# moskewcz/boda

Measured on AMD Instinct MI355X. Metric: effective TFLOP/s (2*M*N*K / time), whole job, higher is better.
Workload: dtype f32

## Files before the change

boda_amd/csrc/kernels/sgemm_big_f32.hip:

```cpp

#ifndef __HIPCC_RTC__
#include <hip/hip_runtime.h>
#endif

typedef float f32x16 __attribute__((ext_vector_type(16)));
typedef float f32x4 __attribute__((ext_vector_type(4)));
typedef unsigned u32x2 __attribute__((ext_vector_type(2)));
#ifndef GROUP_I
#define GROUP_I 8
#endif
#ifndef BKS
#define BKS 8
#endif
#ifndef PF
#define PF 2
#endif
#ifndef TBI
#define TBI 256
#endif
#ifndef TBJ
#define TBJ 256
#endif
#ifndef WI
#define WI 2
#endif
#ifndef WJ
#define WJ 4
#endif
#ifndef MINW
#define MINW 1
#endif
#ifndef MULPRIO
#define MULPRIO 1
#endif
#ifndef STGPRIO
#define STGPRIO 0
#endif
#ifndef NSTG
#define NSTG 4
#endif

struct gemm_args_t {
  float const *I; float const *J; float *D; float const *bias;
  int Mi, Nj, K;
  int ldI, ldJ, ldD;
  int C, H, W, OH, OW;
  int tiles_i, tiles_j;
  int splitk, kt_per;
  float *ws; long ws_slab;
  unsigned I_bytes, J_bytes;
  unsigned D_bytes;
  int out_ctot, out_coff;
  int const *ktab; int ktab_n;
  long bsI, bsJ, bsD;
};

namespace {
constexpr int kNMW = WI * WJ;
static_assert(kNMW == 8 || kNMW == 4, "eight (or four) multiplying waves");
constexpr int kTI = TBI / (WI * 32), kTJ = TBJ / (WJ * 32);
static_assert(TBI % (WI * 32) == 0 && TBJ % (WJ * 32) == 0 && (kTI == 4 || kTI == 2 || kTI == 1) && (kTJ == 2 || kTJ == 1), "wave tile: 4 | 2 | 1 row blocks x 2 | 1 column blocks");
constexpr int kLDI = TBI + 4, kLDJ = TBJ + 4;
constexpr int kImgI = BKS * kLDI, kImgJ = BKS * kLDJ, kImg2 = kImgI + kImgJ;
constexpr int kNLI = BKS * (TBI / 4) / 256, kNLJ = BKS * (TBJ / 4) / 256;
static_assert((BKS * (TBI / 4)) % 256 == 0 && (BKS * (TBJ / 4)) % 256 == 0, "whole float4 units per staging thread");
constexpr int kKK = BKS / 2;
constexpr int kU = (NSTG == 3) ? 3 * PF : ((PF > NSTG) ? PF : NSTG);
constexpr int kD = NSTG - 1;
static_assert(NSTG == 3 || NSTG == 4, "NSTG: 3 | 4");
constexpr int kOOB = (int)0x80000000;
static_assert(BKS % 4 == 0 && (PF == 2 || PF == 4), "BKS % 4 == 0, PF: 2 | 4");
typedef __amdgpu_buffer_rsrc_t rsrc_t;
__device__ __forceinline__ rsrc_t make_rsrc(float const *p, unsigned bytes) { return __builtin_amdgcn_make_buffer_rsrc((void *)p, 0, (int)bytes, 0x00020000); }
__device__ __forceinline__ f32x4 bload4(rsrc_t r, int voff, int soff) { return __builtin_bit_cast(f32x4, __builtin_amdgcn_raw_buffer_load_b128(r, voff, soff, 0)); }
}

#if (TBI / (WI * 32)) == 4
typedef f32x4 avec_t;
#elif (TBI / (WI * 32)) == 2
typedef float2 avec_t;
#else
typedef float avec_t;
#endif
#if (TBJ / (WJ * 32)) == 2
typedef float2 bvec_t;
#else
typedef float bvec_t;
#endif
namespace {
__device__ __forceinline__ float vget(f32x4 const &v, int i) { return v[i]; }
__device__ __forceinline__ float vget(float2 const &v, int i) { return i ? v.y : v.x; }
__device__ __forceinline__ float vget(float const &v, int) { return v; }
}

extern "C" __global__ __launch_bounds__((kNMW + 4) * 64, MINW) void KNAME(gemm_args_t const p) {
  __shared__ __attribute__((aligned(16))) float sm[NSTG * kImg2];
  int const lane = threadIdx.x & 63;
  int const wave = __builtin_amdgcn_readfirstlane(threadIdx.x >> 6);
  bool const stager = wave >= kNMW;

  int tile_i, tile_j;
  {
    int const bid = blockIdx.x, nb = p.tiles_i * p.tiles_j;
    int const q = nb >> 3, rr = nb & 7, xcd = bid & 7, idx = bid >> 3;
    int const nid = ((xcd < rr) ? xcd * (q + 1) : rr * (q + 1) + (xcd - rr) * q) + idx;
    int const group_sz = GROUP_I * p.tiles_j, gid = nid / group_sz, first_i = gid * GROUP_I;
    int const gsz = min(p.tiles_i - first_i, GROUP_I), in_g = nid - gid * group_sz;
    tile_i = first_i + in_g % gsz; tile_j = in_g / gsz;
  }
  int const i0 = tile_i * TBI, j0 = tile_j * TBJ;
  int const nkt = (p.K + BKS - 1) / BKS;
  int const nkt_pad = (nkt + kU - 1) / kU * kU;

  if (stager) {
#if STGPRIO
    __builtin_amdgcn_s_setprio(STGPRIO);
#endif
    int const tid = threadIdx.x - kNMW * 64;
    rsrc_t const rI = make_rsrc(p.I, p.I_bytes), rJ = make_rsrc(p.J, p.J_bytes);
    int goffI[kNLI], goffJ[kNLJ], loffI[kNLI], loffJ[kNLJ], krowI[kNLI], krowJ[kNLJ];
#pragma unroll
    for (int n = 0; n < kNLI; ++n) {
      int const c = tid + n * 256, kr = c / (TBI / 4), x = 4 * (c % (TBI / 4));
      krowI[n] = kr; loffI[n] = kr * kLDI + x;
      goffI[n] = (i0 + x < p.Mi) ? ((kr * p.ldI + i0 + x) * 4) : kOOB;
    }
#pragma unroll
    for (int n = 0; n < kNLJ; ++n) {
      int const c = tid + n * 256, kr = c / (TBJ / 4), x = 4 * (c % (TBJ / 4));
      krowJ[n] = kr; loffJ[n] = kImgI + kr * kLDJ + x;
      goffJ[n] = (j0 + x < p.Nj) ? ((kr * p.ldJ + j0 + x) * 4) : kOOB;
// ... 26 lines not shown
#pragma unroll
        for (int n = 0; n < kNLJ; ++n) { lstoreJ(n, (u + kD) % NSTG, ringJ[(u + kD) % PF][n]); ringJ[(u + kD) % PF][n] = gloadJ(n, kb + u + kD + PF); }
        asm volatile("s_waitcnt lgkmcnt(%0)\n s_barrier" :: "n"(kNLI + kNLJ) : "memory");
      }
    }
    return;
  }

#if MULPRIO
  __builtin_amdgcn_s_setprio(MULPRIO);
#endif
  int const wi = wave / WJ, wj = wave % WJ;
  float const *const a_base = sm + (lane >> 5) * kLDI + wi * (kTI * 32) + kTI * (lane & 31);
  float const *const b_base = sm + kImgI + (lane >> 5) * kLDJ + wj * (kTJ * 32) + kTJ * (lane & 31);
  f32x16 acc[kTI][kTJ];
#pragma unroll
  for (int t = 0; t < kTI; ++t)
#pragma unroll
    for (int u = 0; u < kTJ; ++u)
#pragma unroll
      for (int r = 0; r < 16; ++r) acc[t][u][r] = 0.f;

  asm volatile("s_barrier" ::: "memory");
  avec_t a[2]; bvec_t b[2];
  a[0] = *reinterpret_cast<avec_t const *>(a_base); b[0] = *reinterpret_cast<bvec_t const *>(b_base);
  static_assert(kKK % 2 == 0, "an even number of k pairs per step (the operand double buffer carries over from step to step)");
  for (int kb = 0; kb < nkt_pad; kb += kU) {
#pragma unroll
    for (int s = 0; s < kU; ++s) {
      float const *const A = a_base + (s % NSTG) * kImg2, *const B = b_base + (s % NSTG) * kImg2;
      float const *const An = a_base + ((s + 1) % NSTG) * kImg2, *const Bn = b_base + ((s + 1) % NSTG) * kImg2;
#pragma unroll
      for (int kk = 0; kk < kKK; ++kk) {
        if (kk + 1 < kKK) { a[(kk + 1) & 1] = *reinterpret_cast<avec_t const *>(A + (kk + 1) * 2 * kLDI); b[(kk + 1) & 1] = *reinterpret_cast<bvec_t const *>(B + (kk + 1) * 2 * kLDJ); }
#if NSTG == 4
        else { a[0] = *reinterpret_cast<avec_t const *>(An); b[0] = *reinterpret_cast<bvec_t const *>(Bn); }
#endif
        __builtin_amdgcn_sched_barrier(0);
        avec_t const ca = a[kk & 1]; bvec_t const cb = b[kk & 1];
#pragma unroll
        for (int t = 0; t < kTI; ++t)
#pragma unroll
          for (int u = 0; u < kTJ; ++u) acc[t][u] = __builtin_amdgcn_mfma_f32_32x32x2f32(vget(ca, t), vget(cb, u), acc[t][u], 0, 0, 0);
        __builtin_amdgcn_sched_barrier(0);
      }
#if NSTG == 4
      asm volatile("s_barrier" ::: "memory");
#else
      asm volatile("s_waitcnt lgkmcnt(0)\n s_barrier" ::: "memory");
      a[0] = *reinterpret_cast<avec_t const *>(An); b[0] = *reinterpret_cast<bvec_t const *>(Bn);
#endif
    }
  }

  {
    rsrc_t const rD = make_rsrc(p.D, p.D_bytes);
    int const j = j0 + wj * (kTJ * 32) + kTJ * (lane & 31);
    int const il = i0 + wi * (kTI * 32) + kTI * 4 * (lane >> 5);
#pragma unroll
    for (int t = 0; t < kTI; ++t)
#pragma unroll
      for (int r = 0; r < 16; ++r) {
        int const i = il + kTI * ((r & 3) + 8 * (r >> 2)) + t;
        int const off = ((i < p.Mi) && (j < p.Nj)) ? ((i * p.ldD + j) * 4) : kOOB;
#if (TBJ / (WJ * 32)) == 2
        float2 const v = float2{acc[t][0][r], acc[t][1][r]};
        __builtin_amdgcn_raw_buffer_store_b64(__builtin_bit_cast(u32x2, v), rD, off, 0, 0);
#else
        float const v = acc[t][0][r];
        __builtin_amdgcn_raw_buffer_store_b32(__builtin_bit_cast(unsigned, v), rD, off, 0, 0);
#endif
      }
  }
}
```

boda_amd/csrc/native_internal.h:

```cpp
#pragma once
#include "native_kernels.h"
#include <algorithm>
#include <cstdlib>
#include <sstream>

namespace bodahip {

struct gemm_args_t {
  float const *I; float const *J; float *D; float const *bias;
  int Mi, Nj, K;
  int ldI, ldJ, ldD;
  int C, H, W, OH, OW;
  int tiles_i, tiles_j;
  int splitk, kt_per;
  float *ws; long ws_slab;
  unsigned I_bytes, J_bytes;
  unsigned D_bytes;
  int out_ctot, out_coff;
  void const *ktab; int ktab_n;
  long bsI, bsJ, bsD;
};
struct chain_args_t : gemm_args_t {
  float const *I2; float const *bias2; float *Dmid;
  int M2; unsigned I2_bytes, Dmid_bytes;
};
static_assert(sizeof(gemm_args_t) == 176, "gemm_args_t is declared with this size by every kernel source (and by set_kernel_source's text)");

struct kernel_t { hipModule_t mod = nullptr; hipFunction_t func = nullptr; int occ = 0; };

struct native_kernels_t::impl_t {
  std::map<string, kernel_t> kernels;
  std::map<string, string> tune;
  void *ws = nullptr; size_t ws_bytes = 0;
  bool ws_used = false;
  std::vector<void *> ws_retired;
// ... 62 lines not shown
  float *w0; float *w1; float *w2; float *w3;
  float *ws;
  float *outs[8];
  long n;
  int B, C, HW, N;
  int slab, nslabs;
  int quads;
  int step_img, step_pel;
  float fN, eps, maf, omm, unb;
};
static_assert(sizeof(bn_args_t) == 13 * 8 + 8 * 8 + 8 + 9 * 4 + 5 * 4, "bn_args_t is declared with this layout by kernels/bn_f32.hip");
struct bn_launch_t { plan_t p; int op = 0; };
struct bn_plan_t { std::vector<bn_launch_t> ls; double algo_bytes = 0; size_t ws_bytes = 0; };
bn_plan_t plan_bn(bn_op_t const &b);
string bn_plan_desc(bn_op_t const &b, bn_plan_t const &bp);

struct rows_args_t {
  void const *filts; void const *in; void *out; float const *bias;
  int n_img, oc; unsigned filts_bytes, in_bytes, out_bytes; int out_ctot, out_coff; int n_chunks, rows_per_chunk; float lrn_alpha, lrn_beta, lrn_k;
};

struct sgemm_split_t { uint32_t m_main = 0; string tail_tile; double t_single = 0, t_split = 0; };
static char const *const kBigTile = "256x256x16x2x4x1x1x32x2";
struct sgemm_part_t { uint32_t m0 = 0, rows = 0, n0 = 0, cols = 0; string tile; };
struct set_member_in_t { conv_geom_t g; bool patch_filts, pool; int grp_pad; };
struct set_layout_t { std::vector<int> in_set, alone, variant_of; std::vector<plan_t const *> variants; std::vector<string> vkeys; int minw = 8; string skey; };

extern char const *const k_src_conv_nhwc_bf16_ptr, *const k_src_conv_nhwc_patch_bf16_ptr, *const k_src_winograd_f32_ptr;
bool parse_tile(string const &s, tile_cfg_t &c);
void launch(native_host_t *host, kernel_t &k, gemm_args_t &a, tile_cfg_t const &c);
plan_t plan_sgemm(uint32_t M, uint32_t N, uint32_t K, int num_cus, string const &tile, bool bf16 = false, int batch = 1, bool allow_big = true);
bool plan_patch_bf16(conv_geom_t const &g, int num_cus, plan_t &p);
plan_t plan_conv_nhwc(conv_geom_t const &g, int num_cus, string const &tile, bool out_f32, int grp_pad = 0, bool allow_split = true, bool res = false);
plan_t plan_conv_nhwc_patch(conv_geom_t const &g, int num_cus, string const &tile_arg, bool out_f32, bool pool = false);
bool plan_conv_nhwc_rows(conv_geom_t const &g, post_ops_t const &post, int num_cus, plan_t &p, string *why = nullptr);
bool rows_auto(conv_geom_t const &g, int num_cus, string const &tile);
bool apply_post_ops(op_base_t const &op, conv_geom_t &g, post_ops_t &post, char const *what);
bool plan_ipconv_dma(conv_geom_t const &g, int num_cus, plan_t &p);
plan_t plan_conv(conv_geom_t const &g, int num_cus, string const &tile, bool bf16 = false, string const &k1s = string(), bool allow_splitk = true, bool exact = true);
plan_t plan_bconv_in(conv_geom_t const &g, int num_cus, string const &tile, bool zinp = false);
plan_t plan_bconv_filts(conv_geom_t const &g, int num_cus, string const &tile);
plan_t plan_bconv_filts_biases(conv_geom_t const &g, int num_cus, string const &tile);
plan_t plan_bconv_in_bf16(conv_geom_t const &g, int num_cus, string const &tile, bool zinp = false);
plan_t plan_bconv_fb_bf16(conv_geom_t const &g, int num_cus, string const &tile);
plan_t plan_bconv_slab_sum();
plan_t plan_bconv_biases();
long bconv_in_tiles(conv_geom_t const &g, int BJ);
// ... 22 lines not shown
```

boda_amd/csrc/native_kernels.cc:

```cpp
#include "native_internal.h"

namespace bodahip {

#include "kernels_embed.inc"

native_kernels_t::native_kernels_t(native_host_t *host_) : impl(new impl_t), host(host_) {
  if (char const *e = getenv("BODAHIP_SGEMM_TILE")) impl->tune["sgemm_tile"] = e;
  if (char const *e = getenv("BODAHIP_CONV_TILE")) impl->tune["conv_tile"] = e;
  if (char const *e = getenv("BODAHIP_K1_STREAM")) impl->tune["k1_stream"] = e;
  if (char const *e = getenv("BODAHIP_CONV_ALGO")) impl->tune["conv_algo"] = e;
  if (char const *e = getenv("BODAHIP_EXACT")) impl->tune["exact"] = e;
}
native_kernels_t::~native_kernels_t() {
  if (impl->ts_bytes && impl->ws) {
    char const *e = getenv("BODAHIP_CBIG_TSTAMP"); string fn = e ? string(e) : string(); if (fn.size() > 5 && fn.substr(fn.size() - 5) == ":late") fn.resize(fn.size() - 5);
    std::vector<unsigned long long> h(impl->ts_bytes / 8);
    if (!fn.empty() && hipDeviceSynchronize() == hipSuccess && hipMemcpy(h.data(), (char *)impl->ws + impl->ts_off, impl->ts_bytes, hipMemcpyDeviceToHost) == hipSuccess) {
      if (FILE *f = fopen(fn.c_str(), "a")) { fprintf(f, "%s\n", impl->ts_hdr.c_str());
        for (size_t w = 0; w < h.size() / 16; ++w) { for (int e2 = 0; e2 < 16; ++e2) fprintf(f, "%llu ", h[w * 16 + e2]); fprintf(f, "\n"); } fclose(f); }
    }
  }
  for (auto &kv : impl->kernels) { if (kv.second.mod) (void)hipModuleUnload(kv.second.mod); }
  if (impl->wino_mod) (void)hipModuleUnload(impl->wino_mod);
  if (impl->ws) (void)hipFree(impl->ws);
// ... 185 lines not shown
}

static ktab_t get_rtab(native_kernels_t::impl_t *impl, native_host_t *host, conv_geom_t const &g) {
  string const key = "rows:" + std::to_string(g.C) + "," + std::to_string(g.H) + "," + std::to_string(g.W) + "," + std::to_string(g.KH);
  long const R = (long)g.C * g.KH, n = ((R + 63) / 64 + 1) * 64;
  auto it = impl->ktabs.find(key);
  if (it != impl->ktabs.end()) return ktab_t{it->second, (int)n};
  if (host->nh_capturing()) rt_err("graph capture: gather table not built yet -- run the call list once before capturing it");
  std::vector<int> h((size_t)n * 2);
  for (long r = 0; r < n; ++r) {
    if (r < R) { long const ic = r / g.KH, ky = r % g.KH; h[r] = (int)((ic * g.H + ky) * g.W); h[n + r] = (int)ky; }
    else { h[r] = 0; h[n + r] = 1 << 30; }
  }
  void *d = nullptr;
  hip_err_chk(hipMalloc(&d, h.size() * sizeof(int)), "hipMalloc(rtab)");
  hip_err_chk(hipMemcpyAsync(d, h.data(), h.size() * sizeof(int), hipMemcpyHostToDevice, host->nh_stream()), "hipMemcpyAsync(rtab)");
  hip_err_chk(hipStreamSynchronize(host->nh_stream()), "hipStreamSynchronize");
  impl->ktabs.emplace(key, d);
  return ktab_t{d, (int)n};
}

string tune_of(native_kernels_t::impl_t *impl, char const *key) { auto t = impl->tune.find(key); return (t == impl->tune.end()) ? string() : t->second; }

static void sgemm_parts(native_kernels_t *nk, native_kernels_t::impl_t *impl, native_host_t *host, float const *a, float const *b, float *c, uint32_t M, uint32_t N, uint32_t K, std::vector<sgemm_part_t> const &parts) {
  if ((uint64_t)K * M * 4 > 0x80000000ull || (uint64_t)K * N * 4 > 0x80000000ull || (uint64_t)M * N * 4 >= 0x7ffffff0ull) unsup_err("hip_sgemm: operands / c of 2 GiB or more are not supported (32-bit buffer offsets)");
  uint32_t grid = 0; bool first = true;
  for (sgemm_part_t const &q : parts) {
    plan_t const p = plan_sgemm(q.rows, q.cols, K, host->nh_num_cus(), q.tile, false);
    kernel_t &k = get_kernel(impl, host, p);
    gemm_args_t ga; memset(&ga, 0, sizeof(ga));
    ga.I = a + q.m0; ga.J = b + q.n0; ga.D = c + (size_t)q.m0 * N + q.n0; ga.bias = nullptr;
    ga.Mi = (int)q.rows; ga.Nj = (int)q.cols; ga.K = (int)K; ga.ldI = (int)M; ga.ldJ = (int)N; ga.ldD = (int)N;
    ga.I_bytes = (unsigned)(((uint64_t)K * M - q.m0) * 4); ga.J_bytes = (unsigned)(((uint64_t)K * N - q.n0) * 4); ga.D_bytes = (unsigned)((((uint64_t)q.rows - 1) * N + q.cols) * 4);
    ga.tiles_i = (int)((q.rows + p.cfg.BI - 1) / p.cfg.BI); ga.tiles_j = (int)((q.cols + p.cfg.BJ - 1) / p.cfg.BJ); ga.splitk = 1;
    launch(host, k, ga, p.cfg);
    grid += (uint32_t)ga.tiles_i * ga.tiles_j;
    if (first) { nk->last_launch.kernel = p.kname; nk->last_launch.cfg = p.cfg; nk->last_launch.block = p.cfg.threads(); first = false; }
  }
  nk->last_launch.grid = grid; nk->last_launch.flops = 2.0 * M * N * K; nk->last_launch.algo_bytes = 4.0 * ((double)K * M + (double)K * N + (double)M * N);
}

void native_kernels_t::sgemm(float const *a, float const *b, float *c, uint32_t M, uint32_t N, uint32_t K, bool bf16, bool half) {
  if (!M || !N) return;
  size_t const esz = half ? 2 : 4;
  if (half && bf16) unsup_err("hip_sgemm_bf16: half-typed tensors are not supported (bf16 OPERANDS are made from float tensors)");
  if (!K) { hip_err_chk(hipMemsetAsync(c, 0, (size_t)M * N * esz, host->nh_stream()), "hipMemsetAsync"); return; }
  if (M > 0x7fffffffu || N > 0x7fffffffu || K > 0x7fffffffu) unsup_err("hip_sgemm: dims exceed int32");
  string tile_for;
  if (char const *e = getenv("BODAHIP_SGEMM_TILE_FOR")) {
    string const key = std::to_string(M) + "="; string const v = e; size_t const at = (";" + v).find(";" + key);
    if (M == N && N == K && at != string::npos) { size_t const b = at + key.size(), en = v.find(';', b); tile_for = v.substr(b, en == string::npos ? string::npos : en - b); }
  }
  if (!bf16 && !half && tune_of(impl, "sgemm_tile").empty() && tile_for.empty() && M % 4 == 0 && N % 4 == 0) {
    std::vector<sgemm_part_t> parts;
    if (!parse_parts_env(M, N, K, parts)) parts = plan_sgemm_parts(M, N, K, host->nh_num_cus());
    if (!parts.empty()) { sgemm_parts(this, impl, host, a, b, c, M, N, K, parts); return; }
  }
  if (!bf16 && !half && tune_of(impl, "sgemm_tile").empty() && tile_for.empty()) tile_for = sgemm_wide_tile(M, N, K, host->nh_num_cus());
  if (!bf16 && !half && tune_of(impl, "sgemm_tile").empty() && tile_for.empty()) {
// ... 14 lines not shown
        grid += (uint32_t)ga.tiles_i * ga.tiles_j;
        if (!part) { last_launch.kernel = p.kname; last_launch.cfg = p.cfg; last_launch.block = p.cfg.threads(); }
      }
      last_launch.grid = grid; last_launch.flops = 2.0 * M * N * K; last_launch.algo_bytes = 4.0 * ((double)K * M + (double)K * N + (double)M * N);
      return;
    }
  }
  plan_t p = plan_sgemm(M, N, K, host->nh_num_cus(), tile_for.empty() ? tune_of(impl, "sgemm_tile") : tile_for, bf16, 1, !half);
  if (half) {
    if (p.cfg.SPLITK > 1) unsup_err("hip_sgemm: split-K tiles are not supported for half-typed tensors");
    p.kname = "bodahip_sgemm_f16s"; p.defs.push_back("-DHALF=1");
  }
  tile_cfg_t const &cfg = p.cfg;
  kernel_t &k = get_kernel(impl, host, p);
  gemm_args_t ga; memset(&ga, 0, sizeof(ga));
  ga.I = a; ga.J = b; ga.D = c; ga.bias = nullptr;
  ga.Mi = (int)M; ga.Nj = (int)N; ga.K = (int)K; ga.ldI = (int)M; ga.ldJ = (int)N; ga.ldD = (int)N;
  if ((uint64_t)K * M * 4 > 0x80000000ull || (uint64_t)K * N * 4 > 0x80000000ull) unsup_err("hip_sgemm: operands larger than 2 GiB are not supported (32-bit buffer offsets)");
  ga.I_bytes = (unsigned)((uint64_t)K * M * esz); ga.J_bytes = (unsigned)((uint64_t)K * N * esz);
  if ((uint64_t)M * N * 4 >= 0x7ffffff0ull) unsup_err("hip_sgemm: c of 2 GiB or more is not supported (32-bit store offsets, masked lanes use offset 2^31)");
  ga.D_bytes = (unsigned)((uint64_t)M * N * esz);
  ga.tiles_i = (int)((M + cfg.BI - 1) / cfg.BI); ga.tiles_j = (int)((N + cfg.BJ - 1) / cfg.BJ);
  setup_splitk(impl, host, ga, cfg, (size_t)M * N);
  launch(host, k, ga, cfg);
  if (cfg.SPLITK > 1) reduce_splitk(impl, host, ga, (long)M * N, false, false, 1, 1);
  last_launch.kernel = p.kname; last_launch.cfg = cfg; last_launch.grid = (uint32_t)ga.tiles_i * ga.tiles_j * cfg.SPLITK; last_launch.block = cfg.threads();
  last_launch.flops = 2.0 * M * N * K; last_launch.algo_bytes = (double)esz * ((double)K * M + (double)K * N + (double)M * N);
}

static void launch_patch16(native_kernels_t::impl_t *impl, native_host_t *host, plan_t const &p, kernel_t &k, gemm_args_t &ga, float const *filts,
                           conv_geom_t const &g, size_t ws_off) {
  int const taps = g.KH * g.KW, ncg = (g.C + 7) / 8;
  size_t const fbytes = (size_t)ncg * taps * g.OC * 16;
  if (fbytes >= 0x7ffffff0ull) unsup_err("hip_conv_bf16: re-laid-out filters of 2 GiB or more");
  ensure_ws(impl, host, ws_off + fbytes);
  plan_t fp; fp.patch16 = true; fp.bf16 = true; fp.kname = "bodahip_filt_bf16"; fp.defs = {"-DFILT_ONLY=1"};
  kernel_t &fk = get_kernel(impl, host, fp);
  gemm_args_t fa; memset(&fa, 0, sizeof(fa));
  fa.I = filts; fa.D = (float *)((char *)impl->ws + ws_off); fa.Mi = g.OC; fa.C = g.C; fa.K = taps;
  void *fparams[] = {&fa};
  long const nchunks = (long)ncg * taps * g.OC;
  hip_err_chk(host->nh_launch(fk.func, (uint32_t)((nchunks + 255) / 256), 1, 256, fparams), "hipModuleLaunchKernel(filt_bf16)");
  ga.I = (float const *)((char *)impl->ws + ws_off); ga.I_bytes = (unsigned)fbytes;
  void *params[] = {&ga};
  hip_err_chk(host->nh_launch(k.func, (uint32_t)(ga.tiles_i * ga.tiles_j), 1, (uint32_t)p.cfg.threads(), params), "hipModuleLaunchKernel(conv_patch_bf16)");
}

// ... 562 lines not shown
```

boda_amd/csrc/native_plan.cc:

```cpp
#include "native_internal.h"

namespace bodahip {

bool parse_tile(string const &s, tile_cfg_t &c) {
  int v[11] = {0, 0, 0, 0, 0, 0, 0, 0, 0, 0, 0}; int n = 0; string cur;
  for (size_t i = 0; i <= s.size(); ++i) {
    if (i == s.size() || s[i] == 'x' || s[i] == ':') { if (cur.empty() || n >= 11) return false; v[n++] = atoi(cur.c_str()); cur.clear(); }
    else if (s[i] >= '0' && s[i] <= '9') cur.push_back(s[i]); else return false;
  }
  if (n < 5) return false;
  c.BI = v[0]; c.BJ = v[1]; c.BK = v[2]; c.WI = v[3]; c.WJ = v[4]; c.MINW = (n >= 6) ? v[5] : 1; c.SPLITK = (n >= 7) ? v[6] : 1; c.MT = (n >= 8) ? v[7] : 32; c.PF = (n >= 9) ? v[8] : 1; c.SW = (n >= 10) ? v[9] : 0; c.KHO = (n >= 11) ? v[10] : 0;
  return true;
}
static void check_cfg(tile_cfg_t const &c, bool gather, bool patch = false) {
  int const nt = c.WI * c.WJ * 64;
  bool ok = c.BI > 0 && c.BJ > 0 && c.BK > 0 && c.WI > 0 && c.WJ > 0 && nt <= 1024 && c.threads() <= 1024 && (c.MT == 32 || c.MT == 16) && (c.BI % (c.WI * c.MT) == 0) && (c.BJ % (c.WJ * c.MT) == 0) &&
            (c.BK % 2 == 0) && (c.MT == 32 || c.BK % 4 == 0) && (c.BI % 4 == 0) && (c.BJ % 4 == 0);
  if (gather) ok = ok && ((c.BK * c.BJ) % nt == 0);
  if (gather) ok = ok && (nt % c.BJ == 0) && (c.BJ % 64 == 0);
  ok = ok && c.SPLITK >= 1 && c.SPLITK <= 64 && c.MINW >= 1 && (c.PF == 1 || c.PF == 2 || c.PF == 4 || c.PF == 6 || c.PF == 8);
  ok = ok && c.KHO >= 0 && c.KHO <= 64 && (c.KHO <= 1 || (c.SPLITK == 1 && c.SW == 0));
  if (c.PF > 2) ok = ok && ((long)c.PF * c.BK * (c.BI + c.BJ) / nt <= 192);
  int const accs = (c.BI / (c.WI * c.MT)) * (c.BJ / (c.WJ * c.MT));
  ok = ok && accs * (c.MT == 32 ? 16 : 4) <= 256;
// ... 803 lines not shown
    if (force && atoi(force) == 64) { if (t64 < best) { best = t64; sp.m_main = m_main; sp.tail_tile = kTail64; } continue; }
    if (t128 < best) { best = t128; sp.m_main = m_main; sp.tail_tile = "128x128x16x2x2x2"; }
    if (t64 < best) { best = t64; sp.m_main = m_main; sp.tail_tile = kTail64; }
  }
  sp.t_split = best;
  return sp;
}

string sgemm_wide_tile(uint32_t M, uint32_t N, uint32_t K, long cus) {
  if (M % 4 || N % 4 || K < 512 || getenv("BODAHIP_NO_SGEMM_256X128")) return string();
  if (char const *e = getenv("BODAHIP_SGEMM_BIG")) { if (string(e) == "off") return string(); }
  long const t256 = (long)((M + 255) / 256) * ((N + 255) / 256), t128 = (long)((M + 255) / 256) * ((N + 127) / 128);
  double const eff = (double)t128 / (double)(((t128 + cus - 1) / cus) * cus);
  return (t256 >= cus && eff >= 0.95) ? string("256x128x8x3x4x1") : string();
}

bool parse_parts_env(uint32_t M, uint32_t N, uint32_t K, std::vector<sgemm_part_t> &out) {
  char const *e = getenv("BODAHIP_SGEMM_PARTS"); if (!e || M != N || N != K) return false;
  string const v = e, key = std::to_string(M) + ":"; size_t const at = (";" + v).find(";" + key); if (at == string::npos) return false;
  size_t const b = at + key.size(), en = v.find(';', b); string const spec = v.substr(b, en == string::npos ? string::npos : en - b);
  std::istringstream is(spec); string one;
  while (std::getline(is, one, '/')) {
    sgemm_part_t q; char tl[128];
    if (sscanf(one.c_str(), "%u,%u,%u,%u,%127s", &q.m0, &q.rows, &q.n0, &q.cols, tl) != 5) rt_err("bad BODAHIP_SGEMM_PARTS entry '" + one + "'");
    q.tile = tl; out.push_back(q);
  }
  uint64_t area = 0; for (auto const &q : out) { if (q.m0 % 4 || q.n0 % 4 || q.m0 + q.rows > M || q.n0 + q.cols > N || !q.rows || !q.cols) rt_err("bad BODAHIP_SGEMM_PARTS rectangle"); area += (uint64_t)q.rows * q.cols; }
  if (area != (uint64_t)M * N) rt_err("BODAHIP_SGEMM_PARTS: the rectangles do not add up to c");
  return true;
}

struct sgemm_form_t { char const *tile; int bi, bj, s; double r, lone; };
static sgemm_form_t const kFormQ = {"256x256x16x2x4x1x1x32x2", 256, 256, 1, 1.0, 1.0}, kFormW = {"256x128x8x3x4x1", 256, 128, 2, 1.0127, 0.82}, kFormS = {kStg64, 64, 64, 4, 0.913, 0.5};
static double form_cost(sgemm_form_t const &f, uint32_t rows, uint32_t cols, int cus) {
  long const n = (long)((rows + f.bi - 1) / f.bi) * ((cols + f.bj - 1) / f.bj), per = (long)cus * f.s;
  double const a = (double)f.bi * f.bj / 65536.0, round = f.s * a / f.r;
  if (n <= per) { long const k = (n + cus - 1) / cus; double const eff = (f.s == 1 || k >= f.s) ? 1.0 : f.lone + (1.0 - f.lone) * (double)(k - 1) / (double)(f.s - 1);
                  return (double)k * a / (f.r * eff); }
  if (f.s >= 4) return (double)n / (double)per * round;
  return (double)((n + per - 1) / per) * round;
}
struct sgemm_parts_plan_t { std::vector<sgemm_part_t> parts; double t = 1e30; };
static sgemm_parts_plan_t plan_parts_rec(uint32_t m0, uint32_t rows, uint32_t n0, uint32_t cols, int cus, double ovh, int depth) {
  sgemm_parts_plan_t best;
  for (sgemm_form_t const *f : {&kFormQ, &kFormW, &kFormS}) {
    double const t = form_cost(*f, rows, cols, cus) + ovh;
    if (t < best.t) { best.t = t; sgemm_part_t q; q.m0 = m0; q.rows = rows; q.n0 = n0; q.cols = cols; q.tile = f->tile; best.parts = {q}; }
  }
  if (depth <= 0) return best;
  for (sgemm_form_t const *f : {&kFormQ, &kFormW}) {
    long const per = (long)cus * f->s, tj = (cols + f->bj - 1) / f->bj, ti = (rows + f->bi - 1) / f->bi;
    for (long R = 1; R < ti; ++R) {
      if ((R * tj) % per) continue;
      uint32_t const r1 = (uint32_t)(R * f->bi);
      sgemm_parts_plan_t rest = plan_parts_rec(m0 + r1, rows - r1, n0, cols, cus, ovh, depth - 1);
      double const t = form_cost(*f, r1, cols, cus) + ovh + rest.t;
      if (t < best.t) { best.t = t; sgemm_part_t q; q.m0 = m0; q.rows = r1; q.n0 = n0; q.cols = cols; q.tile = f->tile; best.parts = {q}; best.parts.insert(best.parts.end(), rest.parts.begin(), rest.parts.end()); }
    }
    for (long C = 1; C < tj; ++C) {
      if ((C * ti) % per) continue;
      uint32_t const c1 = (uint32_t)(C * f->bj);
      sgemm_parts_plan_t rest = plan_parts_rec(m0, rows, n0 + c1, cols - c1, cus, ovh, depth - 1);
      double const t = form_cost(*f, rows, c1, cus) + ovh + rest.t;
      if (t < best.t) { best.t = t; sgemm_part_t q; q.m0 = m0; q.rows = rows; q.n0 = n0; q.cols = c1; q.tile = f->tile; best.parts = {q}; best.parts.insert(best.parts.end(), rest.parts.begin(), rest.parts.end()); }
    }
  }
  return best;
}
std::vector<sgemm_part_t> plan_sgemm_parts(uint32_t M, uint32_t N, uint32_t K, int cus) {
  std::vector<sgemm_part_t> none;
  if (getenv("BODAHIP_NO_SGEMM_PARTS") || getenv("BODAHIP_NO_SGEMM_SPLIT") || M % 4 || N % 4 || K < 512 || M < 1024 || N < 1024 || (long)((M + 255) / 256) * ((N + 255) / 256) < cus) return none;
  if (char const *e = getenv("BODAHIP_SGEMM_BIG")) { if (string(e) == "off") return none; }
  if (M % 64 || N % 64) return none;
  double const ovh = 25.7 / (double)K;
  sgemm_parts_plan_t pp = plan_parts_rec(0, M, 0, N, cus, ovh, 3);
  for (uint32_t R = 1024; R < M; R += 1024) {
    sgemm_parts_plan_t const t1 = plan_parts_rec(0, R, 0, N, cus, ovh, 2), t2 = plan_parts_rec(R, M - R, 0, N, cus, ovh, 2);
    if (t1.t + t2.t < pp.t) { pp.t = t1.t + t2.t; pp.parts = t1.parts; pp.parts.insert(pp.parts.end(), t2.parts.begin(), t2.parts.end()); }
  }
  for (uint32_t C = 1024; C < N; C += 1024) {
    sgemm_parts_plan_t const t1 = plan_parts_rec(0, M, 0, C, cus, ovh, 2), t2 = plan_parts_rec(0, M, C, N - C, cus, ovh, 2);
    if (t1.t + t2.t < pp.t) { pp.t = t1.t + t2.t; pp.parts = t1.parts; pp.parts.insert(pp.parts.end(), t2.parts.begin(), t2.parts.end()); }
  }
  if (pp.parts.size() < 2) return none;
  double t_now = std::min(form_cost(kFormQ, M, N, cus), form_cost(kFormW, M, N, cus)) + ovh;
  sgemm_split_t const sp = plan_sgemm_split(M, N, K, cus);
  if (sp.m_main && sgemm_wide_tile(M, N, K, cus).empty()) t_now = std::min(t_now, form_cost(kFormQ, sp.m_main, N, cus) + form_cost(kFormS, M - sp.m_main, N, cus) + 2 * ovh);
  return (pp.t < 0.98 * t_now) ? pp.parts : none;
}



static void check_bconv_cfg(tile_cfg_t const &c, bool filts) {
  int const nt = c.WI * c.WJ * 64;
  bool ok = c.BI > 0 && c.BJ > 0 && c.BK > 0 && c.WI > 0 && c.WJ > 0 && nt <= 1024 && c.MT == 32 && c.BI % (c.WI * 32) == 0 && c.BJ % (c.WJ * 32) == 0 && c.BK % 2 == 0 &&
            nt % c.BJ == 0 && (c.BK * c.BI) % nt == 0 && (c.BK * c.BJ) % nt == 0 && (filts ? (nt % c.BK == 0) : (nt % c.BI == 0)) && c.MINW >= 1 && c.MINW <= 8 &&
            c.SPLITK >= 1 && c.SPLITK <= 32 && (filts || c.SPLITK == 1) && c.PF == 1 && c.SW == 0 && c.KHO == 0;
  int const accs = (c.BI / (c.WI * 32)) * (c.BJ / (c.WJ * 32));
  ok = ok && accs * 16 <= 128 && 2ull * c.BK * (c.BI + 4 + c.BJ + 4) * 4 <= 160 * 1024;
  if (!ok) unsup_err(string(filts ? "hip_bconv_filts" : "hip_bconv_in") + ": unsupported tile configuration " + c.str());
}
static tile_cfg_t bconv_default_cfg(int ni, int BK) {
  tile_cfg_t c; c.BJ = 128; c.BK = BK; c.MINW = 2; c.SPLITK = 1;
  if (ni <= 32) { c.BI = 32; c.WI = 1; c.WJ = 4; } else if (ni <= 64) { c.BI = 64; c.WI = 2; c.WJ = 2; } else { c.BI = 128; c.WI = 2; c.WJ = 2; }
  return c;
}
// ... 274 lines not shown
```

boda_amd/csrc/native_run.cc:

```cpp
#include "native_internal.h"

namespace bodahip {

static conv_geom_t geom_from_dims(dims_t const &f, dims_t const &in, dims_t const &out, dims_t const &stride, dims_t const &in_pad, bool relu) {
  conv_geom_t g;
  g.B = in.dsz("img"); g.C = in.dsz("chan"); g.H = in.dsz("y"); g.W = in.dsz("x");
  g.OC = f.dsz("out_chan"); g.KH = f.dsz("y"); g.KW = f.dsz("x");
  g.SY = stride.dsz("y"); g.SX = stride.dsz("x"); g.PY = in_pad.dsz("y"); g.PX = in_pad.dsz("x");
  g.OH = out.dsz("y"); g.OW = out.dsz("x"); g.relu = relu;
  return g;
}

static bool apply_pool_window(op_base_t const &op, string const &sfx, conv_geom_t &g, char const *what) {
  if (!op.has("nhwc_pool" + sfx) || !op.get_u32("nhwc_pool" + sfx)) return false;
  dims_t const &ks = op.get_dims("pool_sz" + sfx), &pp = op.get_dims("pool_pad" + sfx);
  if (!(g.KH == 1 && g.KW == 1 && g.SY == 1 && g.SX == 1 && g.PY == 0 && g.PX == 0)) rt_err(string(what) + ": fused pooling needs a 1x1 / stride-1 / unpadded convolution");
  g.KH = (int)ks.dsz("y"); g.KW = (int)ks.dsz("x"); g.PY = (int)pp.dsz("y"); g.PX = (int)pp.dsz("x");
  if (g.KH * g.KW < 2 || g.KH * g.KW > 25) unsup_err(string(what) + ": fused pooling windows of 2..25 positions");
  return true;
}

static bool apply_f32_pool(op_base_t const &op, conv_geom_t &g, char const *what) {
  if (!op.has("hip_pool") || !op.get_u32("hip_pool")) return false;
  dims_t const &ks = op.get_dims("pool_sz"), &st = op.get_dims("pool_stride");
// ... 77 lines not shown
  auto const ht = op.str_vals.find("hip_tile");
  string const tile = (tile_arg.empty() && ht != op.str_vals.end()) ? ht->second : tile_arg;
  plan_t p; string log, s2d;
  (void)op_zinp_flag(op);
  (void)op_seed_var_flag(op);
  (void)op_img_shards_flag(op);
  bool const nhwc_res = op_nhwc_residual_flag(op);
  native_func_t const *f = op.has_func_name() ? find_native_func(op.get_func_name()) : nullptr;
  if (f && !f->of_type(t)) f = nullptr;
  std::vector<native_func_t const *> const of_t = native_funcs_of_type(t);
  if (!f && of_t.empty()) rt_err("prebuild: op type '" + t + "' has no native kernel");
  func_family_t const fam = f ? f->family : of_t[0]->family;
  int const member = f ? f->member : 0;
  bool const bf16 = (fam == kFamSgemm && member == 1) || (fam == kFamConv && member == kConvBf16);
  if (fam == kFamSgemm) {
    dims_t const &a = op.get_dims("a"), &b = op.get_dims("b");
    string const wide = (!bf16 && tile.empty() && a.tn != "half") ? sgemm_wide_tile(a.dsz("M"), b.dsz("N"), a.dsz("K"), num_cus) : string();
    sgemm_split_t sp; if (!bf16 && tile.empty() && a.tn != "half" && wide.empty()) sp = plan_sgemm_split(a.dsz("M"), b.dsz("N"), a.dsz("K"), num_cus);
    std::vector<sgemm_part_t> parts; if (!bf16 && tile.empty() && a.tn != "half") parts = plan_sgemm_parts(a.dsz("M"), b.dsz("N"), a.dsz("K"), num_cus);
    if (!parts.empty()) {
      s2d = "parts=" + std::to_string(parts.size());
      for (size_t i = 0; i < parts.size(); ++i) { sgemm_part_t const &q = parts[i];
        p = plan_sgemm(q.rows, q.cols, a.dsz("K"), num_cus, q.tile, false);
        s2d += " [" + std::to_string(q.m0) + "+" + std::to_string(q.rows) + "," + std::to_string(q.n0) + "+" + std::to_string(q.cols) + "]:" + p.cfg.str();
        if (i + 1 < parts.size() && !arch.empty()) compile_plan(p, arch, &log); }
      s2d += " last:";
    }
    else if (!wide.empty()) p = plan_sgemm(a.dsz("M"), b.dsz("N"), a.dsz("K"), num_cus, wide, false);
    else if (sp.m_main) {
      plan_t const tp = plan_sgemm(a.dsz("M") - sp.m_main, b.dsz("N"), a.dsz("K"), num_cus, sp.tail_tile, false);
      p = plan_sgemm(sp.m_main, b.dsz("N"), a.dsz("K"), num_cus, kBigTile, false);
      s2d = "rows<" + std::to_string(sp.m_main) + ":" + p.cfg.str() + "+rest:";
      if (!arch.empty()) compile_plan(p, arch, &log);
      p = tp;
    } else p = plan_sgemm(a.dsz("M"), b.dsz("N"), a.dsz("K"), num_cus, tile, bf16);
    if (a.tn == "half") { s2d.clear(); p = plan_sgemm(a.dsz("M"), b.dsz("N"), a.dsz("K"), num_cus, tile, false, 1, false); p.kname = "bodahip_sgemm_f16s"; p.defs.push_back("-DHALF=1"); }
  }
  else if (fam <= kFamFiltsKmajor) {
    bool const relu = op.has("conv_has_relu") ? (op.get_u32("conv_has_relu") != 0) : true;
    bool const multi = fam == kFamNhwcMulti && member == 0;
    if (fam == kFamNhwcMulti && member == 1) {
      int const n = (int)op.get_dims("multi").dsz("n"); bool const out_f32 = op.get_dims(op.has("out_0") ? "out_0" : "out_0_0").tn == "float";
      std::vector<plan_t> plans; std::vector<double> costs; size_t bytes = 0; string desc;
      for (int m = 0; m < n; ++m) { string const sfx = "_" + std::to_string(m);
        bool const relu_m = op.has("relu_mask") ? (((op.get_u32("relu_mask") >> m) & 1u) != 0) : relu;
        set_member_in_t mi; memset(&mi, 0, sizeof(mi));
        if (op.has("grp" + sfx)) {
// ... 610 lines not shown
```

Before: 145.8.

## Add L-shaped notched sgemm parts, loop-entry alignment padding, and timestamp probes

Lets an sgemm part cover an L shape: the kernel remaps block ids to skip a notch of tiles, so one launch fills whole CU waves and a recursive plan covers the rest. This L-shaped planning is enabled only when an environment variable is set. Unconditionally, the kernel now aligns the main MFMA loop entry to a 64-byte boundary with a few s_nop padding instructions, which is meant to avoid instruction-fetch misalignment in the hot loop. It also adds optional per-block timestamp capture for profiling, gated by a macro and an environment variable.

```diff
diff --git a/boda_amd/csrc/kernels/sgemm_big_f32.hip b/boda_amd/csrc/kernels/sgemm_big_f32.hip
--- a/boda_amd/csrc/kernels/sgemm_big_f32.hip
+++ b/boda_amd/csrc/kernels/sgemm_big_f32.hip
@@ -36,6 +36,9 @@
 #ifndef STGPRIO
 #define STGPRIO 0
 #endif
+#ifndef STAMP
+#define STAMP 0
+#endif
 #ifndef NSTG
 #define NSTG 4
 #endif
@@ -44,7 +47,7 @@
   float const *I; float const *J; float *D; float const *bias;
   int Mi, Nj, K;
   int ldI, ldJ, ldD;
-  int C, H, W, OH, OW;
+  int notch_i, notch_j, W, OH, OW;
   int tiles_i, tiles_j;
   int splitk, kt_per;
   float *ws; long ws_slab;
@@ -69,6 +72,7 @@
 constexpr int kD = NSTG - 1;
 static_assert(NSTG == 3 || NSTG == 4, "NSTG: 3 | 4");
 constexpr int kOOB = (int)0x80000000;
+constexpr int kLoopPad = (kNMW == 4) ? 4 : ((TBI == 256 && TBJ == 256) ? 7 : 8);
 static_assert(BKS % 4 == 0 && (PF == 2 || PF == 4), "BKS % 4 == 0, PF: 2 | 4");
 typedef __amdgpu_buffer_rsrc_t rsrc_t;
 __device__ __forceinline__ rsrc_t make_rsrc(float const *p, unsigned bytes) { return __builtin_amdgcn_make_buffer_rsrc((void *)p, 0, (int)bytes, 0x00020000); }
@@ -98,15 +102,24 @@
   int const lane = threadIdx.x & 63;
   int const wave = __builtin_amdgcn_readfirstlane(threadIdx.x >> 6);
   bool const stager = wave >= kNMW;
+#if STAMP
+  unsigned long long st[5] = {0, 0, 0, 0, 0}; unsigned long long const st_rt0 = __builtin_amdgcn_s_memrealtime();
+  st[0] = __builtin_amdgcn_s_memtime();
+#endif
 
   int tile_i, tile_j;
   {
-    int const bid = blockIdx.x, nb = p.tiles_i * p.tiles_j;
+    int bid = blockIdx.x, ti = p.tiles_i, tj = p.tiles_j, i_off = 0;
+    if (p.notch_i | p.notch_j) {
+      int const n_top = p.notch_i * p.tiles_j;
+      if (bid < n_top) ti = p.notch_i; else { bid -= n_top; i_off = p.notch_i; ti = p.tiles_i - p.notch_i; tj = p.notch_j; }
+    }
+    int const nb = ti * tj;
     int const q = nb >> 3, rr = nb & 7, xcd = bid & 7, idx = bid >> 3;
     int const nid = ((xcd < rr) ? xcd * (q + 1) : rr * (q + 1) + (xcd - rr) * q) + idx;
-    int const group_sz = GROUP_I * p.tiles_j, gid = nid / group_sz, first_i = gid * GROUP_I;
-    int const gsz = min(p.tiles_i - first_i, GROUP_I), in_g = nid - gid * group_sz;
-    tile_i = first_i + in_g % gsz; tile_j = in_g / gsz;
+    int const group_sz = GROUP_I * tj, gid = nid / group_sz, first_i = gid * GROUP_I;
+    int const gsz = min(ti - first_i, GROUP_I), in_g = nid - gid * group_sz;
+    tile_i = i_off + first_i + in_g % gsz; tile_j = in_g / gsz;
   }
   int const i0 = tile_i * TBI, j0 = tile_j * TBJ;
   int const nkt = (p.K + BKS - 1) / BKS;
@@ -179,9 +192,13 @@
       for (int r = 0; r < 16; ++r) acc[t][u][r] = 0.f;
 
   asm volatile("s_barrier" ::: "memory");
+#if STAMP
+  st[1] = __builtin_amdgcn_s_memtime();
+#endif
   avec_t a[2]; bvec_t b[2];
   a[0] = *reinterpret_cast<avec_t const *>(a_base); b[0] = *reinterpret_cast<bvec_t const *>(b_base);
   static_assert(kKK % 2 == 0, "an even number of k pairs per step (the operand double buffer carries over from step to step)");
+  asm volatile(".p2align 6\n .rept %0\n s_nop 0\n .endr" :: "n"(kLoopPad) : "memory");
   for (int kb = 0; kb < nkt_pad; kb += kU) {
 #pragma unroll
     for (int s = 0; s < kU; ++s) {
@@ -210,6 +227,9 @@
     }
   }
 
+#if STAMP
+  st[2] = __builtin_amdgcn_s_memtime();
+#endif
   {
     rsrc_t const rD = make_rsrc(p.D, p.D_bytes);
     int const j = j0 + wj * (kTJ * 32) + kTJ * (lane & 31);
@@ -229,4 +249,20 @@
 #endif
       }
   }
+#if STAMP
+  st[3] = __builtin_amdgcn_s_memtime();
+  asm volatile("s_waitcnt vmcnt(0)" ::: "memory");
+  st[4] = __builtin_amdgcn_s_memtime();
+  unsigned long long const st_rt1 = __builtin_amdgcn_s_memrealtime();
+  if (threadIdx.x == 0 && p.ws) {
+    unsigned long long *const o = reinterpret_cast<unsigned long long *>(p.ws) + 16ull * blockIdx.x;
+#pragma unroll
+    for (int n = 0; n < 5; ++n) o[n] = st[n];
+    o[5] = st_rt0; o[6] = st_rt1;
+    o[7] = __builtin_amdgcn_s_getreg(6 | (11 << 11));
+    o[8] = __builtin_amdgcn_s_getreg(4 | (31 << 11));
+    o[9] = __builtin_amdgcn_s_getreg(20 | (31 << 11));
+    o[10] = (unsigned long long)tile_i << 32 | (unsigned)tile_j;
+  }
+#endif
 }
diff --git a/boda_amd/csrc/native_internal.h b/boda_amd/csrc/native_internal.h
--- a/boda_amd/csrc/native_internal.h
+++ b/boda_amd/csrc/native_internal.h
@@ -10,7 +10,7 @@
   float const *I; float const *J; float *D; float const *bias;
   int Mi, Nj, K;
   int ldI, ldJ, ldD;
-  int C, H, W, OH, OW;
+  union { int C; int notch_i; }; union { int H; int notch_j; }; int W, OH, OW;
   int tiles_i, tiles_j;
   int splitk, kt_per;
   float *ws; long ws_slab;
@@ -119,7 +119,9 @@
 
 struct sgemm_split_t { uint32_t m_main = 0; string tail_tile; double t_single = 0, t_split = 0; };
 static char const *const kBigTile = "256x256x16x2x4x1x1x32x2";
-struct sgemm_part_t { uint32_t m0 = 0, rows = 0, n0 = 0, cols = 0; string tile; };
+struct sgemm_part_t { uint32_t m0 = 0, rows = 0, n0 = 0, cols = 0; string tile; uint32_t nm = 0, nn = 0;
+  bool notched() const { return nm || nn; }
+  uint64_t area() const { return (uint64_t)rows * cols - (notched() ? (uint64_t)(rows - nm) * (cols - nn) : 0); } };
 struct set_member_in_t { conv_geom_t g; bool patch_filts, pool; int grp_pad; };
 struct set_layout_t { std::vector<int> in_set, alone, variant_of; std::vector<plan_t const *> variants; std::vector<string> vkeys; int minw = 8; string skey; };
 
diff --git a/boda_amd/csrc/native_kernels.cc b/boda_amd/csrc/native_kernels.cc
--- a/boda_amd/csrc/native_kernels.cc
+++ b/boda_amd/csrc/native_kernels.cc
@@ -231,19 +231,43 @@
 
 string tune_of(native_kernels_t::impl_t *impl, char const *key) { auto t = impl->tune.find(key); return (t == impl->tune.end()) ? string() : t->second; }
 
-static void sgemm_parts(native_kernels_t *nk, native_kernels_t::impl_t *impl, native_host_t *host, float const *a, float const *b, float *c, uint32_t M, uint32_t N, uint32_t K, std::vector<sgemm_part_t> const &parts) {
+static void *stamp_begin(plan_t const &p, gemm_args_t &ga, uint32_t grid) {
+  if (!getenv("BODAHIP_SGEMM_STAMP") || p.kname != "bodahip_sgemm_big_f32") return nullptr;
+  void *d = nullptr;
+  hip_err_chk(hipMalloc(&d, (size_t)grid * 128), "hipMalloc(stamps)"); hip_err_chk(hipMemset(d, 0, (size_t)grid * 128), "hipMemset(stamps)");
+  ga.ws = (float *)d;
+  return d;
+}
+static void stamp_end(native_host_t *host, void *d, gemm_args_t const &ga, uint32_t grid) {
+  if (!d) return;
+  hip_err_chk(hipStreamSynchronize(host->nh_stream()), "hipStreamSynchronize(stamps)");
+  std::vector<uint64_t> h((size_t)grid * 16 + 5);
+  h[0] = grid; h[1] = (uint64_t)ga.Mi; h[2] = (uint64_t)ga.Nj; h[3] = (uint64_t)ga.K; h[4] = 0;
+  hip_err_chk(hipMemcpy(h.data() + 5, d, (size_t)grid * 128, hipMemcpyDeviceToHost), "hipMemcpy(stamps)"); hip_err_chk(hipFree(d), "hipFree(stamps)");
+  if (FILE *f = fopen(getenv("BODAHIP_SGEMM_STAMP"), "ab")) { fwrite(h.data(), 8, h.size(), f); fclose(f); }
+}
+
+static void sgemm_parts(native_kernels_t *nk,native_kernels_t::impl_t *impl, native_host_t *host, float const *a, float const *b, float *c, uint32_t M, uint32_t N, uint32_t K, std::vector<sgemm_part_t> const &parts) {
   if ((uint64_t)K * M * 4 > 0x80000000ull || (uint64_t)K * N * 4 > 0x80000000ull || (uint64_t)M * N * 4 >= 0x7ffffff0ull) unsup_err("hip_sgemm: operands / c of 2 GiB or more are not supported (32-bit buffer offsets)");
   uint32_t grid = 0; bool first = true;
   for (sgemm_part_t const &q : parts) {
     plan_t const p = plan_sgemm(q.rows, q.cols, K, host->nh_num_cus(), q.tile, false);
     kernel_t &k = get_kernel(impl, host, p);
+    if (q.notched()) {
+      if (!p.big || q.nm % p.cfg.BI || q.nn % p.cfg.BJ || q.nm > q.rows || q.nn > q.cols || !q.area()) rt_err("hip_sgemm: a part's notch must lie on tile boundaries of the staging-wave kernel, inside the part");
+    }
     gemm_args_t ga; memset(&ga, 0, sizeof(ga));
     ga.I = a + q.m0; ga.J = b + q.n0; ga.D = c + (size_t)q.m0 * N + q.n0; ga.bias = nullptr;
     ga.Mi = (int)q.rows; ga.Nj = (int)q.cols; ga.K = (int)K; ga.ldI = (int)M; ga.ldJ = (int)N; ga.ldD = (int)N;
     ga.I_bytes = (unsigned)(((uint64_t)K * M - q.m0) * 4); ga.J_bytes = (unsigned)(((uint64_t)K * N - q.n0) * 4); ga.D_bytes = (unsigned)((((uint64_t)q.rows - 1) * N + q.cols) * 4);
     ga.tiles_i = (int)((q.rows + p.cfg.BI - 1) / p.cfg.BI); ga.tiles_j = (int)((q.cols + p.cfg.BJ - 1) / p.cfg.BJ); ga.splitk = 1;
-    launch(host, k, ga, p.cfg);
-    grid += (uint32_t)ga.tiles_i * ga.tiles_j;
+    uint32_t part_grid = (uint32_t)ga.tiles_i * ga.tiles_j;
+    if (q.notched()) { ga.notch_i = (int)(q.nm / p.cfg.BI); ga.notch_j = (int)(q.nn / p.cfg.BJ); part_grid -= (uint32_t)(ga.tiles_i - ga.notch_i) * (uint32_t)(ga.tiles_j - ga.notch_j); }
+    void *const stamps = stamp_begin(p, ga, part_grid);
+    void *params[] = {&ga};
+    hip_err_chk(host->nh_launch(k.func, part_grid, 1, (uint32_t)p.cfg.threads(), params), "hipModuleLaunchKernel(native, sgemm part)");
+    stamp_end(host, stamps, ga, part_grid);
+    grid += part_grid;
     if (first) { nk->last_launch.kernel = p.kname; nk->last_launch.cfg = p.cfg; nk->last_launch.block = p.cfg.threads(); first = false; }
   }
   nk->last_launch.grid = grid; nk->last_launch.flops = 2.0 * M * N * K; nk->last_launch.algo_bytes = 4.0 * ((double)K * M + (double)K * N + (double)M * N);
@@ -304,7 +328,9 @@
   ga.D_bytes = (unsigned)((uint64_t)M * N * esz);
   ga.tiles_i = (int)((M + cfg.BI - 1) / cfg.BI); ga.tiles_j = (int)((N + cfg.BJ - 1) / cfg.BJ);
   setup_splitk(impl, host, ga, cfg, (size_t)M * N);
+  void *const stamps = (cfg.SPLITK == 1) ? stamp_begin(p, ga, (uint32_t)ga.tiles_i * ga.tiles_j) : nullptr;
   launch(host, k, ga, cfg);
+  stamp_end(host, stamps, ga, (uint32_t)ga.tiles_i * ga.tiles_j);
   if (cfg.SPLITK > 1) reduce_splitk(impl, host, ga, (long)M * N, false, false, 1, 1);
   last_launch.kernel = p.kname; last_launch.cfg = cfg; last_launch.grid = (uint32_t)ga.tiles_i * ga.tiles_j * cfg.SPLITK; last_launch.block = cfg.threads();
   last_launch.flops = 2.0 * M * N * K; last_launch.algo_bytes = (double)esz * ((double)K * M + (double)K * N + (double)M * N);
diff --git a/boda_amd/csrc/native_plan.cc b/boda_amd/csrc/native_plan.cc
--- a/boda_amd/csrc/native_plan.cc
+++ b/boda_amd/csrc/native_plan.cc
@@ -849,10 +849,11 @@
   std::istringstream is(spec); string one;
   while (std::getline(is, one, '/')) {
     sgemm_part_t q; char tl[128];
-    if (sscanf(one.c_str(), "%u,%u,%u,%u,%127s", &q.m0, &q.rows, &q.n0, &q.cols, tl) != 5) rt_err("bad BODAHIP_SGEMM_PARTS entry '" + one + "'");
+    int const nf = sscanf(one.c_str(), "%u,%u,%u,%u,%127[^,],%u,%u", &q.m0, &q.rows, &q.n0, &q.cols, tl, &q.nm, &q.nn);
+    if (nf != 5 && nf != 7) rt_err("bad BODAHIP_SGEMM_PARTS entry '" + one + "'");
     q.tile = tl; out.push_back(q);
   }
-  uint64_t area = 0; for (auto const &q : out) { if (q.m0 % 4 || q.n0 % 4 || q.m0 + q.rows > M || q.n0 + q.cols > N || !q.rows || !q.cols) rt_err("bad BODAHIP_SGEMM_PARTS rectangle"); area += (uint64_t)q.rows * q.cols; }
+  uint64_t area = 0; for (auto const &q : out) { if (q.m0 % 4 || q.n0 % 4 || q.m0 + q.rows > M || q.n0 + q.cols > N || !q.rows || !q.cols || q.nm > q.rows || q.nn > q.cols) rt_err("bad BODAHIP_SGEMM_PARTS rectangle"); area += q.area(); }
   if (area != (uint64_t)M * N) rt_err("BODAHIP_SGEMM_PARTS: the rectangles do not add up to c");
   return true;
 }
@@ -890,6 +891,24 @@
       sgemm_parts_plan_t rest = plan_parts_rec(m0, rows, n0 + c1, cols - c1, cus, ovh, depth - 1);
       double const t = form_cost(*f, rows, c1, cus) + ovh + rest.t;
       if (t < best.t) { best.t = t; sgemm_part_t q; q.m0 = m0; q.rows = rows; q.n0 = n0; q.cols = c1; q.tile = f->tile; best.parts = {q}; best.parts.insert(best.parts.end(), rest.parts.begin(), rest.parts.end()); }
+    }
+  }
+  return best;
+}
+static sgemm_parts_plan_t plan_parts_ell(uint32_t rows, uint32_t cols, int cus, double ovh) {
+  sgemm_parts_plan_t best; double skew = 1e30;
+  for (sgemm_form_t const *f : {&kFormQ, &kFormW}) {
+    long const per = (long)cus * f->s, tj = (cols + f->bj - 1) / f->bj, ti = (rows + f->bi - 1) / f->bi;
+    double const round = f->s * ((double)f->bi * f->bj / 65536.0) / f->r;
+    for (long a = 1; a < ti; ++a) for (long b = 1; b < tj; ++b) {
+      long const nl = ti * tj - (ti - a) * (tj - b);
+      if (nl % per) continue;
+      uint32_t const nm = (uint32_t)(a * f->bi), nn = (uint32_t)(b * f->bj);
+      sgemm_parts_plan_t rest = plan_parts_rec(nm, rows - nm, nn, cols - nn, cus, ovh, 2);
+      double const t = (double)(nl / per) * round + ovh + rest.t, sk = std::fabs(std::log((double)(rows - nm) / (double)(cols - nn)));
+      if (t < best.t - 1e-9 || (t < best.t + 1e-9 && sk < skew)) {
+        best.t = std::min(t, best.t); skew = sk; sgemm_part_t q; q.rows = rows; q.cols = cols; q.tile = f->tile; q.nm = nm; q.nn = nn;
+        best.parts = {q}; best.parts.insert(best.parts.end(), rest.parts.begin(), rest.parts.end()); }
     }
   }
   return best;
@@ -909,6 +928,7 @@
     sgemm_parts_plan_t const t1 = plan_parts_rec(0, M, 0, C, cus, ovh, 2), t2 = plan_parts_rec(0, M, C, N - C, cus, ovh, 2);
     if (t1.t + t2.t < pp.t) { pp.t = t1.t + t2.t; pp.parts = t1.parts; pp.parts.insert(pp.parts.end(), t2.parts.begin(), t2.parts.end()); }
   }
+  if (K >= 2048 && getenv("BODAHIP_SGEMM_ELL")) { sgemm_parts_plan_t const el = plan_parts_ell(M, N, cus, ovh); if (el.t < 0.98 * pp.t) pp = el; }
   if (pp.parts.size() < 2) return none;
   double t_now = std::min(form_cost(kFormQ, M, N, cus), form_cost(kFormW, M, N, cus)) + ovh;
   sgemm_split_t const sp = plan_sgemm_split(M, N, K, cus);
diff --git a/boda_amd/csrc/native_run.cc b/boda_amd/csrc/native_run.cc
--- a/boda_amd/csrc/native_run.cc
+++ b/boda_amd/csrc/native_run.cc
@@ -123,7 +123,7 @@
       s2d = "parts=" + std::to_string(parts.size());
       for (size_t i = 0; i < parts.size(); ++i) { sgemm_part_t const &q = parts[i];
         p = plan_sgemm(q.rows, q.cols, a.dsz("K"), num_cus, q.tile, false);
-        s2d += " [" + std::to_string(q.m0) + "+" + std::to_string(q.rows) + "," + std::to_string(q.n0) + "+" + std::to_string(q.cols) + "]:" + p.cfg.str();
+        s2d += " [" + std::to_string(q.m0) + "+" + std::to_string(q.rows) + "," + std::to_string(q.n0) + "+" + std::to_string(q.cols) + (q.notched() ? " less " + std::to_string(q.nm) + "," + std::to_string(q.nn) : string()) + "]:" + p.cfg.str();
         if (i + 1 < parts.size() && !arch.empty()) compile_plan(p, arch, &log); }
       s2d += " last:";
     }
```

Result: no change. 145.6 (-0.1%).
